# bytedance/DecompDiff

Hardware: AMD Instinct MI355X
Metric: denoising steps/sec (1000-step reverse) per pocket (higher is better)
Workload: dtype f32

## Files before the change

### decompdiff_amd/csrc/dd_api.hip

```cpp
#include <mutex>
#include <thread>
#include <vector>
#include <stddef.h>
#include <stdlib.h>
#include <string.h>
#include <stdio.h>
#include <string>
#include <sys/stat.h>
#include <unistd.h>

#include "dd_kernels.hpp"

namespace dd {

struct Workspace {
  float *xa, *xb, *h, *hb, *ew, *P, *PL, *PB, *P2, *PL2, *PB2, *Ek, *Ev, *Rk, *Rv, *q1bl, *qn, *ql, *ql2, *qlnb, *qb, *A, *Anb, *dxe, *dxb, *ga, *gc, *gr, *h2, *hs;
  int32_t* nbr;
  int32_t* counters;
  size_t total;
};

static inline size_t align64(size_t n) { return (n + 63) & ~(size_t)63; }

static Workspace carve(float* base, int B, int NP, int NL, int K) {
// ... 104 lines not shown
extern int g_tail_variant;
#endif
static bool g_gemm_ksplit_on() { return g_gemm_ksplit != 0; }
struct DevCtx {
  hipStream_t side = nullptr;
  hipEvent_t ev_qa_fork[8], ev_qb_fork[8], ev_fork[9], ev_join[9];
};
static DevCtx g_dev_ctx[16];
static std::mutex g_capture_mutex;
static DevCtx& dev_ctx() {
  int dev = 0;
  if (hipGetDevice(&dev) != hipSuccess || dev < 0 || dev >= 16) dev = 0;
  return g_dev_ctx[dev];
}
#ifndef DD_SIDE_LIN_DEFAULT
#define DD_SIDE_LIN_DEFAULT 0
#endif
#if defined(DD_DEBUG_OPTIONS) && DD_DEBUG_OPTIONS
#define DD_OPT static int
#else
#define DD_OPT static constexpr int
#endif
DD_OPT g_step_fused = 1;
DD_OPT g_step_fold = 1;
DD_OPT g_xup_in_asm = 1;
DD_OPT g_sched = 4;
DD_OPT g_xup_in_pos = 0;
DD_OPT g_fused_max_nl = DD_NL_MAX;
DD_OPT g_defer_pos = 0;
DD_OPT g_lin_with_pb2 = 1;
DD_OPT g_pb_early = 1;
DD_OPT g_q1_in_gemm = 1;
DD_OPT g_l0_tables = 1;
DD_OPT g_head_fused = 1;
DD_OPT g_side_lin = DD_SIDE_LIN_DEFAULT;
static int g_lin_in_node = [] { const char* e = getenv("DD_LIN_IN_NODE"); return e ? (e[0] == '1' ? 1 : (e[0] == '0' ? 0 : -1)) : -1; }();
static int g_lin_proj_main = [] { const char* e = getenv("DD_LIN_PROJ_MAIN"); return e ? (e[0] == '1' ? 1 : 0) : 0; }();
static bool lin_in_node_for(int B, int NL) {
  if (g_lin_in_node >= 0) return g_lin_in_node != 0;
  return (long)B * NL * (NL - 1) < 8L * 256 * 2;
}
DD_OPT g_head_rows_first = 0;
DD_OPT g_heads_early = 1;
static bool uses_lin_in_node(int B, int NL, bool out_fc, bool fused) {
  return fused && !out_fc && lin_in_node_for(B, NL) && g_lin_with_pb2 && !g_side_lin && g_heads_early;
}
DD_OPT g_q_in_pos = 1;
extern int g_pos_waves;
DD_OPT g_p2_in_pos = 0;
static int g_side_low_priority = [] { const char* e = getenv("DD_SIDE_PRIO"); return (e && e[0] == '1') ? 1 : ((e && e[0] == '2') ? 2 : 0); }();
static int g_overlap = 1;
static int ensure_side_stream(DevCtx& dc) {
  if (dc.side) return DD_OK;
  {
    int lo = 0, hi = 0;
    if (hipDeviceGetStreamPriorityRange(&lo, &hi) != hipSuccess) { lo = 0; (void)hipGetLastError(); }
    if (hipStreamCreateWithPriority(&dc.side, hipStreamNonBlocking, g_side_low_priority == 1 ? lo : (g_side_low_priority == 2 ? hi : 0)) != hipSuccess) return DD_ERR_HIP;
  }
  for (int i = 0; i < 8; ++i)
    if (hipEventCreateWithFlags(&dc.ev_qa_fork[i], hipEventDisableTiming) != hipSuccess ||
        hipEventCreateWithFlags(&dc.ev_qb_fork[i], hipEventDisableTiming) != hipSuccess)
      return DD_ERR_HIP;
  for (int i = 0; i < 9; ++i)
    if (hipEventCreateWithFlags(&dc.ev_fork[i], hipEventDisableTiming) != hipSuccess ||
        hipEventCreateWithFlags(&dc.ev_join[i], hipEventDisableTiming) != hipSuccess)
      return DD_ERR_HIP;
// ... 242 lines not shown
  }
  void set_q_in_pos(int l, AttnArgs& pe, AttnArgs& pb) const {
    pe.qhid = w.PL2 + 256; pe.ld_qhid = 1024; pe.lnq = LW(l, DD_PE_lnq); pe.W2q = LW(l, DD_PE_W2qT); pe.b2q = LW(l, DD_PE_b2q);
    pb.qhid = w.PL2 + 896; pb.ld_qhid = 1024; pb.lnq = LW(l, DD_PB_lnq); pb.W2q = LW(l, DD_PB_W2qT); pb.b2q = LW(l, DD_PB_b2q);
  }

  GraphArgs graph_head() const {
    GraphArgs g{};
    g.B = B; g.NP = NP; g.NL = NL; g.K = K;
    g.prot = s->protein_pos; g.prot_stride = 3 * NP; g.lig = s->lig_pos; g.lig_stride = 3 * NL;
    g.nbr = w.nbr; g.ew = w.ew;
    g.EW_W1T = GW(DD_G_EW_W1T); g.EW_b1 = GW(DD_G_EW_b1); g.EW_ln = GW(DD_G_EW_ln); g.EW_w2 = GW(DD_G_EW_w2); g.EW_b2 = GW(DD_G_EW_b2);
    g.np_real = s->np_real; g.nl_real = s->nl_real;
    return g;
  }
  GraphArgs graph_at(const float* x) const {
    GraphArgs g = graph_head();
    g.set_block(x);
    return g;
  }
  EmbedArgs embed(int32_t* advance) const {
    EmbedArgs e{};
    e.B = B; e.NP = NP; e.NL = NL; e.nv = num_v(s);
    e.protein_h = s->protein_h; e.protein_pos = s->protein_pos; e.lig_pos = s->lig_pos; e.lig_v = s->lig_v; e.lig_aux = s->lig_aux;
    e.bond = s->lig_bond;
    e.Wl = GW(DD_G_W_lemb); e.bl = GW(DD_G_b_lemb); e.Wb = GW(DD_G_W_bemb); e.bb = GW(DD_G_b_bemb);
    e.h = w.h; e.xa = w.xa; e.xb = w.xb; e.hb = w.hb;
    e.counters = w.counters; e.advance = advance;
    e.bond_rows = (long)B * Eb;
    e.node_blocks = (int)(((long)B * N * 128 + 255) / 256);
    e.blocks = e.node_blocks + (int)((e.bond_rows * 128 + 255) / 256);
    return e;
  }
  Layer0RowsArgs l0_rows() const {
    Layer0RowsArgs r{};
    r.B = B; r.NP = NP; r.NL = NL;
    r.tab = s->l0_tables; r.lig_v = s->lig_v; r.lig_aux = s->lig_aux; r.bond = s->lig_bond;
    r.l0_P = s->l0_P; r.PL = w.PL; r.l0_qn = s->l0_qn; r.qlnb = w.qlnb; r.PB = w.PB; r.qb = w.qb;
    r.pl_width = plw;
    r.atom_f4 = (long)B * NL * l0_atom_f4(plw);
    r.blocks = (int)((r.atom_f4 + (long)B * Eb * DD_L0_BOND_F4 + 255) / 256);
    return r;
  }
  int launch_head_rows(bool l0, int32_t* advance, hipStream_t sx) const {
    const Layer0RowsArgs r = l0_rows();
    return dd::launch_head_rows(embed(advance), l0 ? &r : nullptr, sx);
  }
  AssembleArgs assemble(int l, const float* x, float* q1) const {
    AssembleArgs a{};
    a.x = x; a.PB = w.PB; a.PL = w.PL; a.Wgp = LW(l, DD_BL_Wgp);
    a.B = B; a.NP = NP; a.NL = NL;
    a.narrow = narrow;
    a.Ek = w.Ek; a.Ev = w.Ev; a.q1 = narrow ? nullptr : q1; a.Rk = w.Rk; a.Rv = w.Rv;
    a.dxe = w.dxe; a.dxb = w.dxb;
    a.fw = no_wait();
    return a;
  }
};

#if defined(DD_DEBUG_OPTIONS) && DD_DEBUG_OPTIONS
static int forward_tail(const Fwd& f, DevCtx& dc, hipStream_t st, StepFold* fold, bool two_streams) {
  const dd_sampler* s = f.s;
  const Workspace& w = f.w;
  const int B = f.B, NP = f.NP, NL = f.NL, N = f.N, nE = f.nE, L = s->num_layers;
  int32_t* flags = w.counters + DD_NUM_COUNTERS;
  auto FL = [&](int l, int fl) { return (l * DD_FLAGS_PER_LAYER + fl) * DD_FLAG_STRIDE; };
  if (two_streams) DD_TRY(ensure_side_stream(dc));
  const bool l0 = g_l0_tables && s->l0_tables && s->l0_P && s->l0_qn && s->nl_real == nullptr;
  int32_t* advance = (fold && fold->advance) ? s->step_counter : nullptr;

  bool head_join = false;
  if (two_streams) {
    if (hipEventRecord(dc.ev_fork[8], st) != hipSuccess || hipStreamWaitEvent(dc.side, dc.ev_fork[8], 0) != hipSuccess) return DD_ERR_HIP;
    DD_TRY(launch_graph(f.graph_head(), dc.side));
    if (hipEventRecord(dc.ev_join[8], dc.side) != hipSuccess) return DD_ERR_HIP;
    head_join = true;
    DD_TRY(f.launch_head_rows(l0, advance, st));
  } else {
    DD_TRYP(DD_PROF_MISC, f.launch_head_rows(l0, advance, st));
    DD_TRYP(DD_PROF_MISC, launch_graph(f.graph_head(), st));
  }
  if (!l0) {
// ... 116 lines not shown

static int forward_impl(const dd_sampler* s, hipStream_t st, StepFold* fold = nullptr, const ModelOpts& mo = ModelOpts()) {
  const dd_bond_head* bh = mo.bh;
  const dd_node_out* no = mo.no;
  DD_TRY(check_shapes(s));
  DD_TRY(check_node_out(no, s));
  DD_TRY(check_blocks(s, mo.num_blocks));
  const bool pre_att = is_pre_att(bh);
  const bool out_fc = no != nullptr;
  const Fwd f(s);
  const Workspace& w = f.w;
  const int B = f.B, NP = f.NP, NL = f.NL, N = f.N;
  const int LB = s->num_layers, L = mo.num_blocks * LB;
  DevCtx& dc = dev_ctx();

  float* xcur = w.xa;
  float* xnext = w.xb;
  float* hcur = w.h;
  const bool fused = g_fuse && NL <= g_fused_max_nl && g_dbg_clock == nullptr;
  const bool overlap = fused && g_overlap && g_prof == nullptr && LB <= 8;
  auto ev = [](int l) { return l & 7; };
#if defined(DD_DEBUG_OPTIONS) && DD_DEBUG_OPTIONS
  if (out_fc && (g_sched >= 5 || g_side_lin)) return DD_ERR_UNSUPPORTED_SHAPE;
  if (mo.num_blocks > 1 && (g_sched >= 5 || g_side_lin)) return DD_ERR_UNSUPPORTED_SHAPE;
  if (fused && !pre_att && !f.narrow && g_sched >= 5 && L <= DD_FLAG_LAYERS && g_q1_in_gemm && g_gemm_ksplit_on() && g_q_in_pos && g_head_fused &&
      g_xup_in_asm && !g_xup_in_pos)
    return forward_tail(f, dc, st, fold, overlap);
#endif
  if (out_fc && !fused) return DD_ERR_UNSUPPORTED_SHAPE;
  if (overlap) DD_TRY(ensure_side_stream(dc));

  const bool l0 = fused && g_l0_tables && g_q1_in_gemm && g_gemm_ksplit_on() && s->l0_tables && s->l0_P && s->l0_qn &&
                  s->nl_real == nullptr;
  int32_t* advance = (fold && fold->advance) ? s->step_counter : nullptr;
  bool head_join = false;
  if (overlap && g_head_fused) {
    if (hipEventRecord(dc.ev_fork[8], st) != hipSuccess || hipStreamWaitEvent(dc.side, dc.ev_fork[8], 0) != hipSuccess) return DD_ERR_HIP;
    if (g_head_rows_first) DD_TRYP(DD_PROF_MISC, f.launch_head_rows(l0, advance, st));
    DD_TRYP(DD_PROF_MISC, launch_graph(f.graph_head(), dc.side));
    if (hipEventRecord(dc.ev_join[8], dc.side) != hipSuccess) return DD_ERR_HIP;
    head_join = true;
    if (!g_head_rows_first) DD_TRYP(DD_PROF_MISC, f.launch_head_rows(l0, advance, st));
  } else {
    DD_TRYP(DD_PROF_MISC, launch_embed(f.embed(advance), st));
    if (l0) DD_TRYP(DD_PROF_MISC, launch_layer0_rows(f.l0_rows(), st));
    hipStream_t gs = st;
    if (overlap) {
      if (hipEventRecord(dc.ev_fork[8], st) != hipSuccess || hipStreamWaitEvent(dc.side, dc.ev_fork[8], 0) != hipSuccess) return DD_ERR_HIP;
      gs = dc.side;
    }
    const GraphArgs g = f.graph_at(w.xa);
    DD_TRYP(DD_PROF_MISC, launch_knn(g, gs));
    DD_TRYP(DD_PROF_MISC, launch_edge_weights(g, gs));
    if (overlap) {
      if (hipEventRecord(dc.ev_join[8], dc.side) != hipSuccess) return DD_ERR_HIP;
      head_join = true;
    }
  }
  int pending_join = -1;
  bool heads_done = false;
  const bool lin_in_node = uses_lin_in_node(B, NL, out_fc, fused);
  struct DeferredPos { bool armed; AttnArgs pe, pb; float *xcur, *xnext; int layer; bool xup; } dpos;
  dpos.armed = false;
  auto flush_pos = [&]() -> int {
    if (!dpos.armed) return DD_OK;
    dpos.armed = false;
    if (hipStreamWaitEvent(dc.side, dc.ev_fork[ev(dpos.layer)], 0) != hipSuccess) return DD_ERR_HIP;
    int rc = launch_attn2_pos(dpos.pe, dpos.pb, dc.side);
    if (rc == DD_OK && !dpos.xup) rc = launch_xupdate(dpos.xcur, w.dxe, w.dxb, B, NP, NL, dpos.xnext, dc.side);
    if (rc != DD_OK) return rc;
    if (hipEventRecord(dc.ev_join[ev(dpos.layer)], dc.side) != hipSuccess) return DD_ERR_HIP;
    pending_join = ev(dpos.layer);
    return DD_OK;
  };
  const float* xup_prev = nullptr;
  for (int l = 0; l < L && fused; ++l) {
    const bool last = l + 1 == L;
    const float* const anb_prev = (lin_in_node && l > 0) ? f.anb_buf(l - 1) : nullptr;
// ... 8 lines not shown
        j.add(f.add_anb(f.n1(ll, hsrc), anb_new, true));
        j.add(f.add_anb(f.l1(ll, hsrc), anb_new, false));
      }
      return j.launch(sx);
    };
    const bool ahead = overlap && g_sched >= 1;
    const bool ahead_split = overlap && g_sched >= 2;
    const bool ahead_b2 = overlap && g_sched >= 3 && g_q1_in_gemm && g_gemm_ksplit_on();
    const bool two_joins = ahead_b2 && g_sched >= 4;
    const bool proj_main = lin_in_node && g_lin_proj_main && two_joins && ahead_split;
    const bool pb_early = g_pb_early && g_lin_with_pb2 && !ahead && !lin_in_node;
    const bool l0_here = l0 && l == 0;
    if (pb_early && l > 0) DD_TRYP(DD_PROF_GEMM, launch_batch1_part(l, 1, st, hcur, nullptr));
    else if (!(ahead && l > 0) && !l0_here) DD_TRYP(DD_PROF_GEMM, launch_batch1(l, st));
    const bool q1_in_gemm = g_q1_in_gemm && g_gemm_ksplit_on();
    auto launch_b2 = [&](int ll, hipStream_t sx) -> int { return f.launch_queries(ll, q1_in_gemm, sx); };
    const bool b2_ahead = ahead_b2 && q1_in_gemm && l > 0;
    bool b1_joined = false;
    if (q1_in_gemm && !b2_ahead) {
      if (ahead && l > 0) {
        if (hipStreamWaitEvent(st, dc.ev_join[ev(l)], 0) != hipSuccess) return DD_ERR_HIP;
        b1_joined = true;
      }
      if (!l0_here) DD_TRYP(DD_PROF_GEMM, launch_b2(l, st));
    }
    DD_TRY(flush_pos());
    if (pending_join >= 0) {
      if (hipStreamWaitEvent(st, dc.ev_join[pending_join], 0) != hipSuccess) return DD_ERR_HIP;
      pending_join = -1;
    }
    const bool late_join = two_joins && b2_ahead && !b1_joined;
    if (ahead && l > 0 && !b1_joined && hipStreamWaitEvent(st, late_join ? dc.ev_qb_fork[ev(l)] : dc.ev_join[ev(l)], 0) != hipSuccess)
      return DD_ERR_HIP;
    AssembleArgs as = f.assemble(l, xcur, q1_in_gemm ? nullptr : w.q1bl);
    as.xprev = xup_prev; as.xout = xup_prev ? xcur : nullptr;
    DD_TRYP(DD_PROF_ASSEMBLE, launch_bl_assemble(as, st));
    xup_prev = nullptr;
    if (l > 0 && l % LB == 0) DD_TRYP(DD_PROF_MISC, launch_graph(f.graph_at(xcur), st));
    if (!q1_in_gemm) DD_TRYP(DD_PROF_GEMM, launch_b2(l, st));
    if (head_join) {
      if (hipStreamWaitEvent(st, dc.ev_join[8], 0) != hipSuccess) return DD_ERR_HIP;
      head_join = false;
    }
    if (late_join && hipStreamWaitEvent(st, dc.ev_join[ev(l)], 0) != hipSuccess) return DD_ERR_HIP;
    {
      AttnArgs ne = f.attn_ne(l, xcur, l0_here), nb = f.attn_nb(l, xcur);
      if (lin_in_node) {
        ne.out = hcur; ne.lin_W = f.LW(l, DD_W_lin); ne.lin_b = f.LW(l, DD_b_lin); ne.lin_add = anb_prev;
        nb.out = f.anb_buf(l); nb.lin_W = f.LW(l, DD_W_lin);
      }
      DD_TRYP(DD_PROF_ATTN_BL, launch_attn2_node(ne, nb, f.attn_bl(l, xcur), st));
    }
    if (ahead_split && !last && hipEventRecord(dc.ev_qa_fork[ev(l + 1)], st) != hipSuccess) return DD_ERR_HIP;
    const bool side_lin = g_side_lin && ahead_split && ahead_b2 && !last;
    float* const hold = hcur;
    GemmArgs lin_dup;
    if (out_fc) {
      NodeOutArgs na{w.A, w.Anb, hcur, hcur, no->layer[l % LB], B, NP, NL};
      DD_TRYP(DD_PROF_GEMM, launch_node_out_fc(na, st));
    } else if (!lin_in_node) {
      GemmArgs g = f.lin(l, hcur, w.Anb);
      if (side_lin) {
        float* hnew = (hcur == w.h) ? w.h2 : w.h;
        g.Y = hnew; g.acc_src = hold;
        lin_dup = g; lin_dup.Y = w.hs;
        hcur = hnew;
      } else if (hcur != w.h) {
        g.Y = w.h; g.acc_src = hold;
// ... 843 lines not shown
  if (mode != 0 && mode != 1 && mode != 3) return DD_ERR_BAD_ARG;
  dd::g_fuse = (mode == 1 || mode == 3) ? 1 : 0;
  dd::g_overlap = mode == 1 ? 1 : 0;
  return DD_OK;
}

namespace dd { extern int g_pos_g_mode; extern int g_gemm_ksplit; extern int g_attn_waves; extern int g_attn_persist; extern int g_pos_waves; extern int g_bl_first; extern int g_gemm_xcd; }
#if defined(DD_DEBUG_OPTIONS) && DD_DEBUG_OPTIONS
extern "C" int dd_queue_error(const dd_sampler* s, void* stream, int* code) {
  if (!s || !s->workspace || !code) return DD_ERR_BAD_ARG;
  dd::Workspace w = dd::carve(s->workspace, s->B, s->NP, s->NL, s->K);
  int32_t v = 0;
  if (hipMemcpyAsync(&v, w.counters + dd::DD_NUM_COUNTERS + dd::DD_FLAG_ERR, sizeof(v), hipMemcpyDeviceToHost, (hipStream_t)stream) != hipSuccess ||
      hipStreamSynchronize((hipStream_t)stream) != hipSuccess)
    return DD_ERR_HIP;
  *code = (int)v;
  if (v != 0 && hipMemsetAsync(w.counters + dd::DD_NUM_COUNTERS + dd::DD_FLAG_ERR, 0, sizeof(v), (hipStream_t)stream) != hipSuccess) return DD_ERR_HIP;
  return DD_OK;
}
#endif

extern "C" int dd_debug_node_split(int B, int NP, int NL, int K) { return dd::node_split_lookup(B, NP, NL, K); }

extern "C" int dd_debug_schedule(void) { return dd::g_p2_in_pos ? 1 : 0; }

extern "C" int dd_debug_set_option(int key, int value) {
  ++g_options_epoch;
  if (key == 0) return dd_debug_set_fusion(value);
#if defined(DD_DEBUG_OPTIONS) && DD_DEBUG_OPTIONS
  if (key == 1) { dd::g_gemm_ksplit = value ? 1 : 0; return DD_OK; }
  if (key == 3) { dd::g_attn_persist = value ? 1 : 0; return DD_OK; }
  if (key == 24) { dd::g_head_fused = value ? 1 : 0; return DD_OK; }
  if (key == 22) { dd::g_l0_tables = value ? 1 : 0; return DD_OK; }
  if (key == 21) { dd::g_gemm_xcd = value ? 1 : 0; return DD_OK; }
  if (key == 20) { dd::g_step_fold = value ? 1 : 0; return DD_OK; }
  if (key == 19) { dd::g_xup_in_asm = value ? 1 : 0; return DD_OK; }
  if (key == 18) { if (value < 0 || value > 1024) return DD_ERR_BAD_ARG; dd::g_bl_first = value; return DD_OK; }
  if (key == 17) { dd::g_pb_early = value ? 1 : 0; return DD_OK; }
  if (key == 16) { dd::g_lin_with_pb2 = value ? 1 : 0; return DD_OK; }
  if (key == 14) { dd::g_defer_pos = value ? 1 : 0; return DD_OK; }
  if (key == 13) { dd::g_fused_max_nl = value; return DD_OK; }
  if (key == 12) { dd::g_q1_in_gemm = value ? 1 : 0; return DD_OK; }
  if (key == 11) { dd::g_xup_in_pos = value ? 1 : 0; return DD_OK; }
  if (key == 9) { dd::g_q_in_pos = value ? 1 : 0; return DD_OK; }
  if (key == 8) { if (value < 0 || value > 5) return DD_ERR_BAD_ARG; dd::g_sched = value; return DD_OK; }
  if (key == 25) { dd::g_tail_variant = value; return DD_OK; }
  if (key == 27) { dd::g_side_lin = value ? 1 : 0; return DD_OK; }
  if (key == 30) { dd::g_p2_in_pos = value ? 1 : 0; return DD_OK; }
  if (key == 31) { dd::g_pos_g_mode = value & 3; return DD_OK; }
  if (key == 28) { dd::g_heads_early = value ? 1 : 0; return DD_OK; }
  if (key == 32) { dd::g_lin_in_node = value < 0 ? -1 : (value ? 1 : 0); return DD_OK; }
  if (key == 29) { dd::g_head_rows_first = value ? 1 : 0; return DD_OK; }
  if (key == 7) { dd::g_step_fused = value ? 1 : 0; return DD_OK; }
  if (key == 5) { if (value != 2 && value != 4 && value != 8) return DD_ERR_BAD_ARG; dd::g_pos_waves = value; return DD_OK; }
  if (key == 2) { if (value != 8) return DD_ERR_BAD_ARG; dd::g_attn_waves = value; return DD_OK; }
  return DD_ERR_BAD_ARG;
#else
  (void)value;
  return DD_ERR_BAD_ARG;
#endif
}
```

### decompdiff_amd/csrc/dd_graph.hip

```cpp
#include <type_traits>

#include "dd_kernels.hpp"

namespace dd {


__device__ __forceinline__ bool atom_is_real(int n, int NP, int npb, int nlb) { return n < NP ? n < npb : (n - NP) < nlb; }

struct PosView {
  const float* p;
  const float* l;
  int NP;
  __device__ __forceinline__ float get(int n, int c) const { return n < NP ? p[3 * n + c] : l[3 * (n - NP) + c]; }
};
__device__ __forceinline__ PosView pos_view(const GraphArgs& a, int b) {
  return PosView{a.prot + (long)b * a.prot_stride, a.lig + (long)b * a.lig_stride, a.NP};
}
__device__ __forceinline__ PosView block_view(const GraphArgs& a, int b) {
  const float* xb = a.prot + (long)b * (a.NP + a.NL) * 3;
  return PosView{xb, xb + 3 * (long)a.NP, a.NP};
}

template <int CAND>
__device__ __forceinline__ void knn_wave(const PosView& pv, int i, int N, int K, int32_t* __restrict__ nbr_row, bool masked, int npb,
// ... 268 lines not shown
    }
  } else {
    const long idx = (long)(blk - e.node_blocks) * 256 + threadIdx.x;
    if (idx >= e.bond_rows * 128) return;
    const int c = idx & 127;
    const long r = idx >> 7;
    e.hb[idx] = e.Wb[c * 5 + e.bond[r]] + e.bb[c];
  }
}
__global__ __launch_bounds__(256) void k_embed_all(const EmbedArgs e) { embed_block(blockIdx.x, e); }

constexpr int L0_TN = 0, L0_TL = 16 * 640, L0_TB = L0_TL + 16 * 1280, L0_TQN = L0_TB + 5 * 640, L0_TQL = L0_TQN + 16 * 128,
              L0_TQB = L0_TQL + 16 * 128;
template <int PLW>
__device__ __forceinline__ void layer0_rows_block(const unsigned blk, const Layer0RowsArgs& r) {
  const long idx = (long)blk * 256 + threadIdx.x;
  const int NP = r.NP, NL = r.NL, N = NP + NL, Eb = NL * (NL - 1);
  auto combo = [&](long a) { return (r.lig_aux[2 * a + 1] > 0.5f ? 8 : 0) + r.lig_v[a]; };
  const float4* t4 = reinterpret_cast<const float4*>(r.tab);
  if (idx < r.atom_f4) {
    constexpr int PER = l0_atom_f4(PLW), K1 = 160 + PLW / 4, K2 = K1 + 32;
    static_assert(PLW != 1280 || (PER == DD_L0_ATOM_F4 && K1 == 480 && K2 == 512), "wide layout");
    const long a = idx / PER;
    const int k = (int)(idx % PER);
    const int b = (int)(a / NL), i = (int)(a % NL);
    const int c = combo(a);
    const long node = (long)b * N + NP + i;
    if (k < 160) reinterpret_cast<float4*>(r.l0_P + node * 640)[k] = t4[(L0_TN + c * 640) / 4 + k];
    else if (k < K1) reinterpret_cast<float4*>(r.PL + a * 1280)[k - 160] = t4[(L0_TL + c * 1280) / 4 + (k - 160)];
    else if (k < K2) reinterpret_cast<float4*>(r.l0_qn + node * 128)[k - K1] = t4[(L0_TQN + c * 128) / 4 + (k - K1)];
    else reinterpret_cast<float4*>(r.qlnb + a * 128)[k - K2] = t4[(L0_TQL + c * 128) / 4 + (k - K2)];
    return;
  }
  constexpr int PERB = DD_L0_BOND_F4;
  const long j = idx - r.atom_f4;
  const long e = j / PERB;
  if (e >= (long)r.B * Eb) return;
  const int k = (int)(j % PERB);
  const int ty = r.bond[e];
  if (k < 160) {
    reinterpret_cast<float4*>(r.PB + e * 640)[k] = t4[(L0_TB + ty * 640) / 4 + k];
  } else {
    const int b = (int)(e / Eb), t = (int)((e % Eb) / (NL - 1));
    const int c = combo((long)b * NL + t);
    reinterpret_cast<float4*>(r.qb + e * 128)[k - 160] = t4[(L0_TQB + (c * 5 + ty) * 128) / 4 + (k - 160)];
  }
}
template <int PLW>
__global__ __launch_bounds__(256) void k_layer0_rows(const Layer0RowsArgs r) { layer0_rows_block<PLW>(blockIdx.x, r); }

template <int CAND, int KW>
__global__ __launch_bounds__(256, 3) void k_graph(const GraphArgs a) {
  __shared__ unsigned long long sel[4][64];
  __shared__ int32_t srt[4][KW];
  __shared__ __attribute__((aligned(16))) float lw[512];
  ew_stage(lw, a.EW_b1, a.EW_ln, a.EW_w2);
  __syncthreads();
  const int N = a.NP + a.NL, w = threadIdx.x >> 6, lane = threadIdx.x & 63;
  const int centre = (int)blockIdx.x * 4 + w;
  if (centre >= a.B * N) return;
  const int b = centre / N, i = centre % N;
  const bool masked = a.nl_real != nullptr;
  const int npb = masked && a.np_real ? a.np_real[b] : a.NP, nlb = masked ? a.nl_real[b] : a.NL;
  if (masked && !atom_is_real(i, a.NP, npb, nlb)) {
    if (lane < a.K) a.nbr[(long)centre * a.K + lane] = 0;
    return;
  }
  const PosView pv = pos_view(a, b);
  knn_wave<CAND>(pv, i, N, a.K, a.nbr + (long)centre * a.K, masked, npb, nlb, sel[w], srt[w]);
  ew_wave(pv, i, a.K, srt[w], a.EW_W1T, lw, a.EW_b2, a.ew + (long)centre * a.K);
}
template <int PLW>
__global__ __launch_bounds__(256) void k_head_rows(const EmbedArgs e, const Layer0RowsArgs r) {
  const unsigned blk = blockIdx.x;
  if ((int)blk < e.blocks) embed_block(blk, e);
  else layer0_rows_block<PLW>(blk - e.blocks, r);
}

typedef float f32x4a __attribute__((ext_vector_type(4)));
template <bool WIDE>
__global__ __launch_bounds__(256, 2) void k_bl_assemble3(const float* __restrict__ x, const float* __restrict__ PB,
                                                      const float* __restrict__ PL, const float* __restrict__ Wgp ,
                                                      int B, int NP, int NL, float* __restrict__ Ek, float* __restrict__ Ev,
                                                      float* __restrict__ q1, float* __restrict__ Rk, float* __restrict__ Rv,
                                                      int blocks_per_output, const float* __restrict__ xprev,
                                                      const float* __restrict__ dxe, const float* __restrict__ dxb,
                                                      float* __restrict__ xout, const FlagWait fw) {
  if (xprev != nullptr && blockIdx.x == 0) {
    const int n = B * NL * 3;
    for (int idx = threadIdx.x; idx < n; idx += 256) {
      const int bb = idx / (NL * 3), r = idx % (NL * 3);
      const long xi = ((long)bb * (NP + NL) + NP) * 3 + r;
      xout[xi] = xprev[xi] + dxe[idx] + dxb[idx];
    }
  }
  __shared__ __attribute__((aligned(16))) float tab[DD_NGAUSS * 128];
  const int q = blockIdx.x / blocks_per_output;
  if (q < 4) {
    const float4* src = reinterpret_cast<const float4*>(Wgp + q * DD_NGAUSS * 128);
    for (int i = threadIdx.x; i < DD_NGAUSS * 32; i += 256) reinterpret_cast<float4*>(tab)[i] = src[i];
  }
  if (fw.flags != nullptr) dd_wait_flags(fw.flags, fw.idx0, fw.n0, fw.idx1, fw.n1, DD_FLAG_ERR, 300);
  else __syncthreads();
  const int lane = threadIdx.x & 63, mm = lane & 15, cg = lane >> 4;
  const int Eb = NL * (NL - 1), N = NP + NL;
  const long nrows = (long)B * Eb;
  const long tile = (long)(blockIdx.x % blocks_per_output) * 4 + (threadIdx.x >> 6);
  if (tile * 16 >= nrows) return;
  const long e_raw = tile * 16 + mm;
  const bool valid = e_raw < nrows;
  const long e_glob = valid ? e_raw : nrows - 1;
  const int b = e_glob / Eb, e = e_glob % Eb;
  const int t = e / (NL - 1), sp = e % (NL - 1);
  const int s = sp + (sp >= t ? 1 : 0);
  const float* pb = PB + e_glob * 640 + 4 * cg;
  const float* ps = WIDE ? PL + ((long)b * NL + s) * 1280 + 4 * cg : nullptr;
  const float* pt = WIDE ? PL + ((long)b * NL + t) * 1280 + 4 * cg : nullptr;
  auto ld4 = [](const float* p) { return *reinterpret_cast<const float4*>(p); };
  if (WIDE && q == 4) {
    if (q1 != nullptr && valid) {
#pragma unroll
      for (int nt = 0; nt < 8; ++nt) {
        const float4 a0 = ld4(pb + 512 + 16 * nt), a1 = ld4(pt + 1152 + 16 * nt);
        *reinterpret_cast<float4*>(q1 + e_glob * 128 + 4 * cg + 16 * nt) = make_float4(a0.x + a1.x, a0.y + a1.y, a0.z + a1.z, a0.w + a1.w);
      }
    }
    return;
  }
  f32x4a acc[8];
#pragma unroll
  for (int nt = 0; nt < 8; ++nt) {
    if (q < 2) {
      const float4 a0 = ld4(pb + 256 + 128 * q + 16 * nt);
      if constexpr (WIDE) {
        const float4 a1 = ld4(ps + 640 + 256 * q + 16 * nt);
        const float4 a2 = ld4(pt + 768 + 256 * q + 16 * nt);
        acc[nt] = f32x4a{(a0.x + a1.x) + a2.x, (a0.y + a1.y) + a2.y, (a0.z + a1.z) + a2.z, (a0.w + a1.w) + a2.w};
      } else {
        acc[nt] = f32x4a{a0.x, a0.y, a0.z, a0.w};
      }
    } else {
      acc[nt] = f32x4a{0.f, 0.f, 0.f, 0.f};
    }
  }
  float dx, dy, dz;
  if (xprev != nullptr) {
    const float* xl = xprev + ((long)b * N + NP) * 3;
    const float* de = dxe + (long)b * NL * 3;
    const float* db = dxb + (long)b * NL * 3;
    dx = (xl[3 * t] + de[3 * t] + db[3 * t]) - (xl[3 * s] + de[3 * s] + db[3 * s]);
    dy = (xl[3 * t + 1] + de[3 * t + 1] + db[3 * t + 1]) - (xl[3 * s + 1] + de[3 * s + 1] + db[3 * s + 1]);
    dz = (xl[3 * t + 2] + de[3 * t + 2] + db[3 * t + 2]) - (xl[3 * s + 2] + de[3 * s + 2] + db[3 * s + 2]);
  } else {
    const float* xl = x + ((long)b * N + NP) * 3;
    dx = xl[3 * t] - xl[3 * s]; dy = xl[3 * t + 1] - xl[3 * s + 1]; dz = xl[3 * t + 2] - xl[3 * s + 2];
  }
  const float d = sqrtf(dx * dx + dy * dy + dz * dz);
  const float* tb = tab + cg * 128 + mm * 4;
#pragma unroll
  for (int k = 0; k < 5; ++k) {
    const float fk = gauss_feat(d, 4 * k + cg);
    const float4 w0 = *reinterpret_cast<const float4*>(tb + k * 512);
    const float4 w1 = *reinterpret_cast<const float4*>(tb + k * 512 + 64);
    acc[0] = __builtin_amdgcn_mfma_f32_16x16x4f32(w0.x, fk, acc[0], 0, 0, 0);
    acc[1] = __builtin_amdgcn_mfma_f32_16x16x4f32(w0.y, fk, acc[1], 0, 0, 0);
    acc[2] = __builtin_amdgcn_mfma_f32_16x16x4f32(w0.z, fk, acc[2], 0, 0, 0);
    acc[3] = __builtin_amdgcn_mfma_f32_16x16x4f32(w0.w, fk, acc[3], 0, 0, 0);
    acc[4] = __builtin_amdgcn_mfma_f32_16x16x4f32(w1.x, fk, acc[4], 0, 0, 0);
    acc[5] = __builtin_amdgcn_mfma_f32_16x16x4f32(w1.y, fk, acc[5], 0, 0, 0);
    acc[6] = __builtin_amdgcn_mfma_f32_16x16x4f32(w1.z, fk, acc[6], 0, 0, 0);
    acc[7] = __builtin_amdgcn_mfma_f32_16x16x4f32(w1.w, fk, acc[7], 0, 0, 0);
  }
  float* dst = (q == 0 ? Ek : (q == 1 ? Ev : (q == 2 ? Rk : Rv))) + e_glob * 128 + 4 * cg;
  if (valid) {
#pragma unroll
    for (int nt = 0; nt < 8; ++nt)
      *reinterpret_cast<float4*>(dst + 16 * nt) = make_float4(acc[nt][0], acc[nt][1], acc[nt][2], acc[nt][3]);
  }
}

__global__ void k_extract_ligand(const float* __restrict__ x, int B, int NP, int NL, float* __restrict__ out) {
  int idx = blockIdx.x * blockDim.x + threadIdx.x;
  if (idx >= B * NL * 3) return;
  int b = idx / (NL * 3), r = idx % (NL * 3);
  out[idx] = x[((long)b * (NP + NL) + NP) * 3 + r];
}
int launch_extract_ligand(const float* x, int B, int NP, int NL, float* out, hipStream_t st) {
  int n = B * NL * 3;
// ... 48 lines not shown
  if (a.K <= 0 || a.K > DD_KNN_MAX || a.K > N - 1 || N > DD_N_MAX) return DD_ERR_UNSUPPORTED_SHAPE;
  with_cand_class<2, 4, 6, 11, 16, DD_N_MAX / 64>((N + 63) / 64, [&](auto c) {
    constexpr int CAND = decltype(c)::value;
    if (a.K <= 32) hipLaunchKernelGGL((k_graph<CAND, 32>), graph_grid(a), dim3(256), 0, st, a);
    else hipLaunchKernelGGL((k_graph<CAND, 64>), graph_grid(a), dim3(256), 0, st, a);
  });
  DD_CHECK_LAUNCH();
  return DD_OK;
}
int launch_embed(const EmbedArgs& e, hipStream_t st) {
  hipLaunchKernelGGL(k_embed_all, dim3((unsigned)e.blocks), dim3(256), 0, st, e);
  DD_CHECK_LAUNCH();
  return DD_OK;
}
int launch_layer0_rows(const Layer0RowsArgs& r, hipStream_t st) {
  if (r.pl_width == 640) hipLaunchKernelGGL(k_layer0_rows<640>, dim3((unsigned)r.blocks), dim3(256), 0, st, r);
  else hipLaunchKernelGGL(k_layer0_rows<1280>, dim3((unsigned)r.blocks), dim3(256), 0, st, r);
  DD_CHECK_LAUNCH();
  return DD_OK;
}
int launch_head_rows(const EmbedArgs& e, const Layer0RowsArgs* r, hipStream_t st) {
  if (r != nullptr && e.nv != DD_NUM_V) return DD_ERR_UNSUPPORTED_SHAPE;
  const dim3 grid((unsigned)(e.blocks + (r ? r->blocks : 0)));
  if (r != nullptr && r->pl_width == 640) hipLaunchKernelGGL(k_head_rows<640>, grid, dim3(256), 0, st, e, *r);
  else hipLaunchKernelGGL(k_head_rows<1280>, grid, dim3(256), 0, st, e, r ? *r : Layer0RowsArgs{});
  DD_CHECK_LAUNCH();
  return DD_OK;
}
int launch_bl_assemble(const AssembleArgs& a, hipStream_t st) {
  if (a.Wgp == nullptr) return DD_ERR_BAD_ARG;
  const long rows = (long)a.B * a.NL * (a.NL - 1);
  const long tiles = (rows + 15) / 16;
  const int bpo = (int)((tiles + 3) / 4);
  if (a.narrow) {
    if (a.q1 != nullptr) return DD_ERR_BAD_ARG;
    hipLaunchKernelGGL(k_bl_assemble3<false>, dim3((unsigned)(bpo * 4)), dim3(256), 0, st, a.x, a.PB, nullptr, a.Wgp, a.B, a.NP, a.NL,
                       a.Ek, a.Ev, nullptr, a.Rk, a.Rv, bpo, a.xprev, a.dxe, a.dxb, a.xout, a.fw);
  } else {
    hipLaunchKernelGGL(k_bl_assemble3<true>, dim3((unsigned)(bpo * (a.q1 ? 5 : 4))), dim3(256), 0, st, a.x, a.PB, a.PL, a.Wgp, a.B, a.NP,
                       a.NL, a.Ek, a.Ev, a.q1, a.Rk, a.Rv, bpo, a.xprev, a.dxe, a.dxb, a.xout, a.fw);
  }
  DD_CHECK_LAUNCH();
  return DD_OK;
}

}

static dd::GraphArgs graph_args(const float* x, int B, int NP, int NL, int K, int32_t* nbr) {
  dd::GraphArgs a{};
  a.B = B; a.NP = NP; a.NL = NL; a.K = K; a.nbr = nbr;
  a.set_block(x);
  return a;
}
extern "C" int dd_knn(const float* x, int B, int N, int K, int32_t* nbr, void* stream) {
  if (!x || !nbr || B <= 0 || N <= 1) return DD_ERR_BAD_ARG;
  if (N > DD_N_MAX || K > DD_KNN_MAX || K > N - 1 || K <= 0) return DD_ERR_UNSUPPORTED_SHAPE;
  return dd::launch_knn(graph_args(x, B, N, 0, K, nbr), (hipStream_t)stream);
}

extern "C" int dd_knn_masked(const float* x, int B, int NP, int NL, int K, const int32_t* np_real, const int32_t* nl_real, int32_t* nbr,
                             void* stream) {
  const int N = NP + NL;
  if (!x || !nbr || !nl_real || B <= 0 || NP < 0 || NL <= 0 || K <= 0 || K > DD_KNN_MAX || K > N - 1 || N > DD_N_MAX) return DD_ERR_BAD_ARG;
  dd::GraphArgs a = graph_args(x, B, NP, NL, K, nbr);
  a.np_real = np_real; a.nl_real = nl_real;
  return dd::launch_knn(a, (hipStream_t)stream);
}

extern "C" int dd_knn_csr(const float* x, const int32_t* ptr, int B, int n, int n_max, int K, int loop, const int64_t* out_off,
                          int64_t E, int64_t* edge_index, void* stream) {
  if (!ptr || !out_off || B <= 0 || n < 0 || E < 0 || K <= 0 || (loop != 0 && loop != 1)) return DD_ERR_BAD_ARG;
  if (K > DD_KNN_MAX) return DD_ERR_UNSUPPORTED_SHAPE;
  if (n == 0 || E == 0) return DD_OK;
// ... 29 lines not shown
```

### decompdiff_amd/csrc/dd_kernels.hpp

```cpp
#pragma once
#include "dd_common.hpp"

namespace dd {

struct FlagWait { const int32_t* flags; int idx0, n0, idx1, n1; };
inline FlagWait no_wait() { return FlagWait{nullptr, -1, 0, -1, 0}; }

struct GemmArgs {
  const float* X; int x_rows_per_b; long x_stride_b; int ldx; int rows;
  const float* W; const float* bias; const float* ln;
  float* Y; int y_rows_per_b; long y_stride_b; int ldy; int ncols; int accumulate;
  const float* X2; int x2_N, x2_NP;
  int x2_Eb, x2_NLm1, x2_ld;
  long long* dbg;
  const float* acc_src;
};
inline GemmArgs gemm_args(const float* X, int x_rows_per_b, long x_stride_b, int ldx, int rows, const float* W,
                          const float* bias, const float* ln, float* Y, int y_rows_per_b, long y_stride_b, int ldy,
                          int ncols, int accumulate) {
  GemmArgs g{X, x_rows_per_b, x_stride_b, ldx, rows, W, bias, ln, Y, y_rows_per_b, y_stride_b, ldy, ncols, accumulate,
             nullptr, 0, 0, 0, 0, 0, nullptr, nullptr};
  return g;
}
enum { DD_FLAG_TICKET = 0, DD_FLAG_LIN = 1, DD_FLAG_TICKET2 = 2, DD_FLAG_PL1 = 3, DD_FLAG_P1Q = 4, DD_FLAG_PBQ = 5, DD_FLAG_PB1R = 6,
// ... 31 lines not shown
int launch_gemm128_batch(const GemmArgs* jobs, int njobs, hipStream_t st);
struct NodeOutArgs { const float* Ae; const float* Ab; const float* h; float* out; const float* blk; int B, NP, NL; };
int launch_node_out_fc(const NodeOutArgs& a, hipStream_t st);

struct GraphArgs {
  int B, NP, NL, K;
  const float* prot; int prot_stride;
  const float* lig; int lig_stride;
  int32_t* nbr;
  float* ew;
  const float *EW_W1T, *EW_b1, *EW_ln, *EW_w2, *EW_b2;
  const int32_t *np_real, *nl_real;
  void set_block(const float* x) { prot = x; lig = x + 3 * (long)NP; prot_stride = lig_stride = 3 * (NP + NL); }
};
int launch_graph(const GraphArgs& a, hipStream_t st);
int launch_knn(const GraphArgs& a, hipStream_t st);
int launch_edge_weights(const GraphArgs& a, hipStream_t st);

struct EmbedArgs {
  int B, NP, NL;
  int nv;
  const float *protein_h, *protein_pos, *lig_pos;
  const int32_t* lig_v;
  const float* lig_aux;
  const int32_t* bond;
  const float *Wl, *bl, *Wb, *bb;
  float *h, *xa, *xb, *hb;
  int32_t *counters, *advance;
  long bond_rows;
  int node_blocks, blocks;
};
constexpr int l0_atom_f4(int pl_width) { return 160 + pl_width / 4 + 32 + 32; }
constexpr int DD_L0_ATOM_F4 = l0_atom_f4(1280);
constexpr int DD_L0_BOND_F4 = 160 + 32;
struct Layer0RowsArgs {
  int B, NP, NL;
  const float* tab;
  const int32_t* lig_v;
  const float* lig_aux;
  const int32_t* bond;
  float *l0_P, *PL, *l0_qn, *qlnb, *PB, *qb;
  long atom_f4;
  int blocks;
  int pl_width;
};
int launch_embed(const EmbedArgs& e, hipStream_t st);
int launch_layer0_rows(const Layer0RowsArgs& r, hipStream_t st);
int launch_head_rows(const EmbedArgs& e, const Layer0RowsArgs* r , hipStream_t st);

struct AssembleArgs {
  const float *x, *PB, *PL, *Wgp;
  int B, NP, NL;
  float *Ek, *Ev, *q1, *Rk, *Rv;
  const float *xprev, *dxe, *dxb;
  float* xout;
  FlagWait fw;
  bool narrow;
};
int launch_bl_assemble(const AssembleArgs& a, hipStream_t st);
int launch_drift_armsca(const float* lig_pos, const int32_t* decomp_index, int B, int NL, float min_d, float max_d,
                        float* grad, int accumulate, int norm_B, hipStream_t st);
int launch_drift_arms_repul(const float* lig_pos, const int32_t* decomp_index, int B, int NL, float max_d, int mode, float* grad,
                            int accumulate, int norm_B, hipStream_t st);
int launch_drift_clash(const float* lig_pos, const float* offset, const float* full_protein_pos, int B, int NL, int NF,
                       float sigma, float gamma, float* grad, int accumulate, const int32_t* nl_real, hipStream_t st);
int launch_extract_ligand(const float* x, int B, int NP, int NL, float* out, hipStream_t st);

enum { M_NE = 0, M_NB = 1, M_BL = 2, M_PE = 3, M_PB = 4 };

struct AttnArgs {
  int B, NP, NL, K;
  const float* x;
  const int32_t* nbr;
  const float* ew;
  const float *kd, *ks, *vd, *vs, *ke, *ve;
  int ld_kd, ld_ks, ld_vd, ld_vs, ld_ke, ld_ve;
  const float* q;
  const float *Akp, *Avp;
  const float *Wakp, *Wavp;
  const float *lnk, *lnv;
  const float* W2k;
  const float* b2v;
  const float* W2v;
  const float *qhid, *lnq, *W2q, *b2q; int ld_qhid;
  int* work_counter;
  const float *W2v16, *b2v16;
  float* out;
  const float* dxe;
  float* x_next;
  const float *Rk, *Rv;
// ... 62 lines not shown
```

Before: 883.8.

## Read layer-0 bond/atom projections directly from tables in assemble kernel

For layer 0, the bond-ligand assemble kernel now indexes the precomputed l0 tables by bond type and atom type instead of reading materialized PB/PL rows. The head-rows kernel therefore writes only the first 64 float4 of each PB row instead of 160, which cuts per-step global write traffic. The assemble kernel is also restructured so coordinate, table-weight and accumulator loads are issued before the shared-memory barrier, overlapping latency. An optional, off-by-default path moves head rows to the side stream. It adds indirect gathers and extra register pressure.

```diff
diff --git a/decompdiff_amd/csrc/dd_api.hip b/decompdiff_amd/csrc/dd_api.hip
--- a/decompdiff_amd/csrc/dd_api.hip
+++ b/decompdiff_amd/csrc/dd_api.hip
@@ -160,6 +160,14 @@
 DD_OPT g_pb_early = 1;
 DD_OPT g_q1_in_gemm = 1;
 DD_OPT g_l0_tables = 1;
+#ifndef DD_L0_INDIRECT_DEFAULT
+#define DD_L0_INDIRECT_DEFAULT 1
+#endif
+#ifndef DD_HEAD_ROWS_SIDE_DEFAULT
+#define DD_HEAD_ROWS_SIDE_DEFAULT 0
+#endif
+DD_OPT g_l0_indirect = DD_L0_INDIRECT_DEFAULT;
+DD_OPT g_head_rows_side = DD_HEAD_ROWS_SIDE_DEFAULT;
 DD_OPT g_head_fused = 1;
 DD_OPT g_side_lin = DD_SIDE_LIN_DEFAULT;
 static int g_lin_in_node = [] { const char* e = getenv("DD_LIN_IN_NODE"); return e ? (e[0] == '1' ? 1 : (e[0] == '0' ? 0 : -1)) : -1; }();
@@ -468,22 +476,23 @@
     e.blocks = e.node_blocks + (int)((e.bond_rows * 128 + 255) / 256);
     return e;
   }
-  Layer0RowsArgs l0_rows() const {
+  Layer0RowsArgs l0_rows(int pb_f4) const {
     Layer0RowsArgs r{};
     r.B = B; r.NP = NP; r.NL = NL;
     r.tab = s->l0_tables; r.lig_v = s->lig_v; r.lig_aux = s->lig_aux; r.bond = s->lig_bond;
     r.l0_P = s->l0_P; r.PL = w.PL; r.l0_qn = s->l0_qn; r.qlnb = w.qlnb; r.PB = w.PB; r.qb = w.qb;
-    r.pl_width = plw;
+    r.pl_width = plw; r.pb_f4 = pb_f4;
     r.atom_f4 = (long)B * NL * l0_atom_f4(plw);
-    r.blocks = (int)((r.atom_f4 + (long)B * Eb * DD_L0_BOND_F4 + 255) / 256);
+    r.blocks = (int)((r.atom_f4 + (long)B * Eb * (pb_f4 + 32) + 255) / 256);
     return r;
   }
-  int launch_head_rows(bool l0, int32_t* advance, hipStream_t sx) const {
-    const Layer0RowsArgs r = l0_rows();
+  int launch_head_rows(bool l0, int32_t* advance, hipStream_t sx, int pb_f4 = 160) const {
+    const Layer0RowsArgs r = l0_rows(pb_f4);
     return dd::launch_head_rows(embed(advance), l0 ? &r : nullptr, sx);
   }
-  AssembleArgs assemble(int l, const float* x, float* q1) const {
+  AssembleArgs assemble(int l, const float* x, float* q1, bool l0_src = false) const {
     AssembleArgs a{};
+    if (l0_src) { a.l0.tab = s->l0_tables; a.l0.bond = s->lig_bond; a.l0.lig_v = s->lig_v; a.l0.lig_aux = s->lig_aux; }
     a.x = x; a.PB = w.PB; a.PL = w.PL; a.Wgp = LW(l, DD_BL_Wgp);
     a.B = B; a.NP = NP; a.NL = NL;
     a.narrow = narrow;
@@ -666,18 +675,22 @@
 
   const bool l0 = fused && g_l0_tables && g_q1_in_gemm && g_gemm_ksplit_on() && s->l0_tables && s->l0_P && s->l0_qn &&
                   s->nl_real == nullptr;
+  const bool l0_indirect = l0 && g_l0_indirect;
+  const int pb_f4 = l0_indirect ? DD_L0_PB_F4 : 160;
+  const bool rows_side = l0_indirect && g_head_rows_side && overlap && g_head_fused;
   int32_t* advance = (fold && fold->advance) ? s->step_counter : nullptr;
   bool head_join = false;
   if (overlap && g_head_fused) {
     if (hipEventRecord(dc.ev_fork[8], st) != hipSuccess || hipStreamWaitEvent(dc.side, dc.ev_fork[8], 0) != hipSuccess) return DD_ERR_HIP;
-    if (g_head_rows_first) DD_TRYP(DD_PROF_MISC, f.launch_head_rows(l0, advance, st));
+    if (g_head_rows_first && !rows_side) DD_TRYP(DD_PROF_MISC, f.launch_head_rows(l0, advance, st, pb_f4));
+    if (rows_side) DD_TRYP(DD_PROF_MISC, f.launch_head_rows(l0, advance, dc.side, pb_f4));
     DD_TRYP(DD_PROF_MISC, launch_graph(f.graph_head(), dc.side));
     if (hipEventRecord(dc.ev_join[8], dc.side) != hipSuccess) return DD_ERR_HIP;
     head_join = true;
-    if (!g_head_rows_first) DD_TRYP(DD_PROF_MISC, f.launch_head_rows(l0, advance, st));
+    if (!g_head_rows_first && !rows_side) DD_TRYP(DD_PROF_MISC, f.launch_head_rows(l0, advance, st, pb_f4));
   } else {
     DD_TRYP(DD_PROF_MISC, launch_embed(f.embed(advance), st));
-    if (l0) DD_TRYP(DD_PROF_MISC, launch_layer0_rows(f.l0_rows(), st));
+    if (l0) DD_TRYP(DD_PROF_MISC, launch_layer0_rows(f.l0_rows(pb_f4), st));
     hipStream_t gs = st;
     if (overlap) {
       if (hipEventRecord(dc.ev_fork[8], st) != hipSuccess || hipStreamWaitEvent(dc.side, dc.ev_fork[8], 0) != hipSuccess) return DD_ERR_HIP;
@@ -752,8 +765,9 @@
     const bool late_join = two_joins && b2_ahead && !b1_joined;
     if (ahead && l > 0 && !b1_joined && hipStreamWaitEvent(st, late_join ? dc.ev_qb_fork[ev(l)] : dc.ev_join[ev(l)], 0) != hipSuccess)
       return DD_ERR_HIP;
-    AssembleArgs as = f.assemble(l, xcur, q1_in_gemm ? nullptr : w.q1bl);
+    AssembleArgs as = f.assemble(l, xcur, q1_in_gemm ? nullptr : w.q1bl, l0_here && l0_indirect);
     as.xprev = xup_prev; as.xout = xup_prev ? xcur : nullptr;
+    if (l0_here && rows_side) as.x_lig = s->lig_pos;
     DD_TRYP(DD_PROF_ASSEMBLE, launch_bl_assemble(as, st));
     xup_prev = nullptr;
     if (l > 0 && l % LB == 0) DD_TRYP(DD_PROF_MISC, launch_graph(f.graph_at(xcur), st));
@@ -1663,6 +1677,8 @@
   if (key == 3) { dd::g_attn_persist = value ? 1 : 0; return DD_OK; }
   if (key == 24) { dd::g_head_fused = value ? 1 : 0; return DD_OK; }
   if (key == 22) { dd::g_l0_tables = value ? 1 : 0; return DD_OK; }
+  if (key == 34) { dd::g_l0_indirect = value ? 1 : 0; return DD_OK; }
+  if (key == 35) { dd::g_head_rows_side = value ? 1 : 0; return DD_OK; }
   if (key == 21) { dd::g_gemm_xcd = value ? 1 : 0; return DD_OK; }
   if (key == 20) { dd::g_step_fold = value ? 1 : 0; return DD_OK; }
   if (key == 19) { dd::g_xup_in_asm = value ? 1 : 0; return DD_OK; }
diff --git a/decompdiff_amd/csrc/dd_graph.hip b/decompdiff_amd/csrc/dd_graph.hip
--- a/decompdiff_amd/csrc/dd_graph.hip
+++ b/decompdiff_amd/csrc/dd_graph.hip
@@ -324,18 +324,18 @@
     else reinterpret_cast<float4*>(r.qlnb + a * 128)[k - K2] = t4[(L0_TQL + c * 128) / 4 + (k - K2)];
     return;
   }
-  constexpr int PERB = DD_L0_BOND_F4;
+  const int PERB = r.pb_f4 + 32;
   const long j = idx - r.atom_f4;
   const long e = j / PERB;
   if (e >= (long)r.B * Eb) return;
   const int k = (int)(j % PERB);
   const int ty = r.bond[e];
-  if (k < 160) {
+  if (k < r.pb_f4) {
     reinterpret_cast<float4*>(r.PB + e * 640)[k] = t4[(L0_TB + ty * 640) / 4 + k];
   } else {
     const int b = (int)(e / Eb), t = (int)((e % Eb) / (NL - 1));
     const int c = combo((long)b * NL + t);
-    reinterpret_cast<float4*>(r.qb + e * 128)[k - 160] = t4[(L0_TQB + (c * 5 + ty) * 128) / 4 + (k - 160)];
+    reinterpret_cast<float4*>(r.qb + e * 128)[k - r.pb_f4] = t4[(L0_TQB + (c * 5 + ty) * 128) / 4 + (k - r.pb_f4)];
   }
 }
 template <int PLW>
@@ -371,13 +371,13 @@
 
 typedef float f32x4a __attribute__((ext_vector_type(4)));
 template <bool WIDE>
-__global__ __launch_bounds__(256, 2) void k_bl_assemble3(const float* __restrict__ x, const float* __restrict__ PB,
+__global__ __launch_bounds__(256, 2) void k_bl_assemble3(const float* __restrict__ xlig, int xstride, const float* __restrict__ PB,
                                                       const float* __restrict__ PL, const float* __restrict__ Wgp ,
                                                       int B, int NP, int NL, float* __restrict__ Ek, float* __restrict__ Ev,
                                                       float* __restrict__ q1, float* __restrict__ Rk, float* __restrict__ Rv,
                                                       int blocks_per_output, const float* __restrict__ xprev,
                                                       const float* __restrict__ dxe, const float* __restrict__ dxb,
-                                                      float* __restrict__ xout, const FlagWait fw) {
+                                                      float* __restrict__ xout, const FlagWait fw, const L0Src l0) {
   if (xprev != nullptr && blockIdx.x == 0) {
     const int n = B * NL * 3;
     for (int idx = threadIdx.x; idx < n; idx += 256) {
@@ -387,65 +387,106 @@
     }
   }
   __shared__ __attribute__((aligned(16))) float tab[DD_NGAUSS * 128];
+#if defined(DD_DEBUG_OPTIONS) && DD_DEBUG_OPTIONS
+  if (fw.flags != nullptr) dd_wait_flags(fw.flags, fw.idx0, fw.n0, fw.idx1, fw.n1, DD_FLAG_ERR, 300);
+#endif
   const int q = blockIdx.x / blocks_per_output;
-  if (q < 4) {
-    const float4* src = reinterpret_cast<const float4*>(Wgp + q * DD_NGAUSS * 128);
-    for (int i = threadIdx.x; i < DD_NGAUSS * 32; i += 256) reinterpret_cast<float4*>(tab)[i] = src[i];
-  }
-  if (fw.flags != nullptr) dd_wait_flags(fw.flags, fw.idx0, fw.n0, fw.idx1, fw.n1, DD_FLAG_ERR, 300);
-  else __syncthreads();
   const int lane = threadIdx.x & 63, mm = lane & 15, cg = lane >> 4;
   const int Eb = NL * (NL - 1), N = NP + NL;
   const long nrows = (long)B * Eb;
   const long tile = (long)(blockIdx.x % blocks_per_output) * 4 + (threadIdx.x >> 6);
-  if (tile * 16 >= nrows) return;
+  const bool live = tile * 16 < nrows;
   const long e_raw = tile * 16 + mm;
   const bool valid = e_raw < nrows;
   const long e_glob = valid ? e_raw : nrows - 1;
   const int b = e_glob / Eb, e = e_glob % Eb;
   const int t = e / (NL - 1), sp = e % (NL - 1);
   const int s = sp + (sp >= t ? 1 : 0);
-  const float* pb = PB + e_glob * 640 + 4 * cg;
-  const float* ps = WIDE ? PL + ((long)b * NL + s) * 1280 + 4 * cg : nullptr;
-  const float* pt = WIDE ? PL + ((long)b * NL + t) * 1280 + 4 * cg : nullptr;
   auto ld4 = [](const float* p) { return *reinterpret_cast<const float4*>(p); };
+  const float *pb, *ps = nullptr, *pt = nullptr;
+  int ty = 0, vs = 0, vt = 0;
+  float fs = 0.f, ft = 0.f;
+  if (l0.tab != nullptr) {
+    ty = l0.bond[e_glob];
+    if constexpr (WIDE) {
+      const long as = (long)b * NL + s, at = (long)b * NL + t;
+      vs = l0.lig_v[as]; fs = l0.lig_aux[2 * as + 1];
+      vt = l0.lig_v[at]; ft = l0.lig_aux[2 * at + 1];
+    }
+  }
+  const float* xl = xprev != nullptr ? xprev + ((long)b * N + NP) * 3 : xlig + (long)b * xstride;
+  const float xt0 = xl[3 * t], xt1 = xl[3 * t + 1], xt2 = xl[3 * t + 2], xs0 = xl[3 * s], xs1 = xl[3 * s + 1], xs2 = xl[3 * s + 2];
+  float et0 = 0.f, et1 = 0.f, et2 = 0.f, es0 = 0.f, es1 = 0.f, es2 = 0.f, bt0 = 0.f, bt1 = 0.f, bt2 = 0.f, bs0 = 0.f, bs1 = 0.f, bs2 = 0.f;
+  if (xprev != nullptr) {
+    const float* de = dxe + (long)b * NL * 3;
+    const float* db = dxb + (long)b * NL * 3;
+    et0 = de[3 * t]; et1 = de[3 * t + 1]; et2 = de[3 * t + 2]; es0 = de[3 * s]; es1 = de[3 * s + 1]; es2 = de[3 * s + 2];
+    bt0 = db[3 * t]; bt1 = db[3 * t + 1]; bt2 = db[3 * t + 2]; bs0 = db[3 * s]; bs1 = db[3 * s + 1]; bs2 = db[3 * s + 2];
+  }
+  static_assert(DD_NGAUSS * 32 == 640, "2.5 float4 per thread");
+  const float4* src = reinterpret_cast<const float4*>(Wgp + (q < 4 ? q : 0) * DD_NGAUSS * 128);
+  const int ti = threadIdx.x;
+  const float4 v0 = src[ti], v1 = src[ti + 256], v2 = src[ti < 128 ? ti + 512 : ti];
+  if (l0.tab != nullptr) {
+    pb = l0.tab + L0_TB + ty * 640 + 4 * cg;
+    if constexpr (WIDE) {
+      ps = l0.tab + L0_TL + ((fs > 0.5f ? 8 : 0) + vs) * 1280 + 4 * cg;
+      pt = l0.tab + L0_TL + ((ft > 0.5f ? 8 : 0) + vt) * 1280 + 4 * cg;
+    }
+  } else {
+    pb = PB + e_glob * 640 + 4 * cg;
+    if constexpr (WIDE) {
+      ps = PL + ((long)b * NL + s) * 1280 + 4 * cg;
+      pt = PL + ((long)b * NL + t) * 1280 + 4 * cg;
+    }
+  }
+  f32x4a acc[8];
+  if (q < 2) {
+    const float* r0 = pb + 256 + 128 * q;
+    const float* r1 = WIDE ? ps + 640 + 256 * q : nullptr;
+    const float* r2 = WIDE ? pt + 768 + 256 * q : nullptr;
+    float4 a0[8], a1[8], a2[8];
+#pragma unroll
+    for (int nt = 0; nt < 8; ++nt) {
+      a0[nt] = ld4(r0 + 16 * nt);
+      if constexpr (WIDE) { a1[nt] = ld4(r1 + 16 * nt); a2[nt] = ld4(r2 + 16 * nt); }
+    }
+#pragma unroll
+    for (int nt = 0; nt < 8; ++nt) {
+      if constexpr (WIDE)
+        acc[nt] = f32x4a{(a0[nt].x + a1[nt].x) + a2[nt].x, (a0[nt].y + a1[nt].y) + a2[nt].y, (a0[nt].z + a1[nt].z) + a2[nt].z,
+                         (a0[nt].w + a1[nt].w) + a2[nt].w};
+      else
+        acc[nt] = f32x4a{a0[nt].x, a0[nt].y, a0[nt].z, a0[nt].w};
+    }
+  } else {
+#pragma unroll
+    for (int nt = 0; nt < 8; ++nt) acc[nt] = f32x4a{0.f, 0.f, 0.f, 0.f};
+  }
+  if (q < 4) {
+    reinterpret_cast<float4*>(tab)[ti] = v0;
+    reinterpret_cast<float4*>(tab)[ti + 256] = v1;
+    if (ti < 128) reinterpret_cast<float4*>(tab)[ti + 512] = v2;
+  }
+  __syncthreads();
+  if (!live) return;
   if (WIDE && q == 4) {
     if (q1 != nullptr && valid) {
 #pragma unroll
       for (int nt = 0; nt < 8; ++nt) {
-        const float4 a0 = ld4(pb + 512 + 16 * nt), a1 = ld4(pt + 1152 + 16 * nt);
-        *reinterpret_cast<float4*>(q1 + e_glob * 128 + 4 * cg + 16 * nt) = make_float4(a0.x + a1.x, a0.y + a1.y, a0.z + a1.z, a0.w + a1.w);
+        const float4 h0 = ld4(pb + 512 + 16 * nt), h1 = ld4(pt + 1152 + 16 * nt);
+        *reinterpret_cast<float4*>(q1 + e_glob * 128 + 4 * cg + 16 * nt) = make_float4(h0.x + h1.x, h0.y + h1.y, h0.z + h1.z, h0.w + h1.w);
       }
     }
     return;
-  }
-  f32x4a acc[8];
-#pragma unroll
-  for (int nt = 0; nt < 8; ++nt) {
-    if (q < 2) {
-      const float4 a0 = ld4(pb + 256 + 128 * q + 16 * nt);
-      if constexpr (WIDE) {
-        const float4 a1 = ld4(ps + 640 + 256 * q + 16 * nt);
-        const float4 a2 = ld4(pt + 768 + 256 * q + 16 * nt);
-        acc[nt] = f32x4a{(a0.x + a1.x) + a2.x, (a0.y + a1.y) + a2.y, (a0.z + a1.z) + a2.z, (a0.w + a1.w) + a2.w};
-      } else {
-        acc[nt] = f32x4a{a0.x, a0.y, a0.z, a0.w};
-      }
-    } else {
-      acc[nt] = f32x4a{0.f, 0.f, 0.f, 0.f};
-    }
   }
   float dx, dy, dz;
   if (xprev != nullptr) {
-    const float* xl = xprev + ((long)b * N + NP) * 3;
-    const float* de = dxe + (long)b * NL * 3;
-    const float* db = dxb + (long)b * NL * 3;
-    dx = (xl[3 * t] + de[3 * t] + db[3 * t]) - (xl[3 * s] + de[3 * s] + db[3 * s]);
-    dy = (xl[3 * t + 1] + de[3 * t + 1] + db[3 * t + 1]) - (xl[3 * s + 1] + de[3 * s + 1] + db[3 * s + 1]);
-    dz = (xl[3 * t + 2] + de[3 * t + 2] + db[3 * t + 2]) - (xl[3 * s + 2] + de[3 * s + 2] + db[3 * s + 2]);
+    dx = (xt0 + et0 + bt0) - (xs0 + es0 + bs0);
+    dy = (xt1 + et1 + bt1) - (xs1 + es1 + bs1);
+    dz = (xt2 + et2 + bt2) - (xs2 + es2 + bs2);
   } else {
-    const float* xl = x + ((long)b * N + NP) * 3;
-    dx = xl[3 * t] - xl[3 * s]; dy = xl[3 * t + 1] - xl[3 * s + 1]; dz = xl[3 * t + 2] - xl[3 * s + 2];
+    dx = xt0 - xs0; dy = xt1 - xs1; dz = xt2 - xs2;
   }
   const float d = sqrtf(dx * dx + dy * dy + dz * dz);
   const float* tb = tab + cg * 128 + mm * 4;
@@ -560,13 +601,16 @@
   const long rows = (long)a.B * a.NL * (a.NL - 1);
   const long tiles = (rows + 15) / 16;
   const int bpo = (int)((tiles + 3) / 4);
+  if (a.l0.tab != nullptr && (!a.l0.bond || (!a.narrow && (!a.l0.lig_v || !a.l0.lig_aux)) || a.fw.flags != nullptr)) return DD_ERR_BAD_ARG;
+  const float* xlig = a.x_lig ? a.x_lig : a.x + 3 * (long)a.NP;
+  const int xstride = a.x_lig ? 3 * a.NL : 3 * (a.NP + a.NL);
   if (a.narrow) {
     if (a.q1 != nullptr) return DD_ERR_BAD_ARG;
-    hipLaunchKernelGGL(k_bl_assemble3<false>, dim3((unsigned)(bpo * 4)), dim3(256), 0, st, a.x, a.PB, nullptr, a.Wgp, a.B, a.NP, a.NL,
-                       a.Ek, a.Ev, nullptr, a.Rk, a.Rv, bpo, a.xprev, a.dxe, a.dxb, a.xout, a.fw);
+    hipLaunchKernelGGL(k_bl_assemble3<false>, dim3((unsigned)(bpo * 4)), dim3(256), 0, st, xlig, xstride, a.PB, nullptr, a.Wgp, a.B, a.NP,
+                       a.NL, a.Ek, a.Ev, nullptr, a.Rk, a.Rv, bpo, a.xprev, a.dxe, a.dxb, a.xout, a.fw, a.l0);
   } else {
-    hipLaunchKernelGGL(k_bl_assemble3<true>, dim3((unsigned)(bpo * (a.q1 ? 5 : 4))), dim3(256), 0, st, a.x, a.PB, a.PL, a.Wgp, a.B, a.NP,
-                       a.NL, a.Ek, a.Ev, a.q1, a.Rk, a.Rv, bpo, a.xprev, a.dxe, a.dxb, a.xout, a.fw);
+    hipLaunchKernelGGL(k_bl_assemble3<true>, dim3((unsigned)(bpo * (a.q1 ? 5 : 4))), dim3(256), 0, st, xlig, xstride, a.PB, a.PL, a.Wgp,
+                       a.B, a.NP, a.NL, a.Ek, a.Ev, a.q1, a.Rk, a.Rv, bpo, a.xprev, a.dxe, a.dxb, a.xout, a.fw, a.l0);
   }
   DD_CHECK_LAUNCH();
   return DD_OK;
diff --git a/decompdiff_amd/csrc/dd_kernels.hpp b/decompdiff_amd/csrc/dd_kernels.hpp
--- a/decompdiff_amd/csrc/dd_kernels.hpp
+++ b/decompdiff_amd/csrc/dd_kernels.hpp
@@ -87,7 +87,7 @@
 };
 constexpr int l0_atom_f4(int pl_width) { return 160 + pl_width / 4 + 32 + 32; }
 constexpr int DD_L0_ATOM_F4 = l0_atom_f4(1280);
-constexpr int DD_L0_BOND_F4 = 160 + 32;
+constexpr int DD_L0_PB_F4 = 64;
 struct Layer0RowsArgs {
   int B, NP, NL;
   const float* tab;
@@ -98,6 +98,13 @@
   long atom_f4;
   int blocks;
   int pl_width;
+  int pb_f4;
+};
+struct L0Src {
+  const float* tab;
+  const int32_t* bond;
+  const int32_t* lig_v;
+  const float* lig_aux;
 };
 int launch_embed(const EmbedArgs& e, hipStream_t st);
 int launch_layer0_rows(const Layer0RowsArgs& r, hipStream_t st);
@@ -111,6 +118,8 @@
   float* xout;
   FlagWait fw;
   bool narrow;
+  L0Src l0;
+  const float* x_lig;
 };
 int launch_bl_assemble(const AssembleArgs& a, hipStream_t st);
 int launch_drift_armsca(const float* lig_pos, const int32_t* decomp_index, int B, int NL, float min_d, float max_d,
```

After: 887.7 (median of 5 runs). Within noise of the previous version (+0.4%).
